# vankxr/qo-100-tools

Hardware: AMD Instinct MI355X
Metric: complex-IQ MSamples/s through 255-tap FIR (higher is better)
Workload: dtype f32

## Files before the change

### include/if_fir_debug.h

```cpp
#ifndef IF_FIR_DEBUG_H
#define IF_FIR_DEBUG_H

#include "if_fir.h"

#ifdef __cplusplus
extern "C" {
#endif

uint8_t if_fir_time_device(if_fir_ctx_t *pCtx, const void *pDevIn, void *pDevOut, uint64_t ullSamples,
                           uint32_t ulWarmup, uint32_t ulReps, float *pfMsPerCall);
uint32_t if_fir_debug_stamps(if_fir_ctx_t *pCtx, uint64_t *pullOut, uint32_t ulWords);
#define IF_FIR_DEBUG_TABLE_FLOATS 21632u
uint32_t if_fir_debug_fft_tables(const float *pfTaps, uint32_t ulTaps, uint32_t bComplexTaps, uint32_t ulDecimation,
                                 uint32_t ulNcoDelta, float *pfOut, uint32_t ulOutFloats);
uint32_t if_fir_debug_fft_tables_bank(const float *pfTaps, uint32_t ulTaps, uint32_t bComplexTaps, uint32_t ulBank, uint32_t ulParity,
                                      float *pfOut, uint32_t ulOutFloats);
uint32_t if_fir_debug_bank_tail(uint32_t ulDecimation, uint32_t bOwnCentres);
uint8_t if_fir_debug_bank_plan(const uint32_t *pulSlots, uint32_t ulChannels, uint32_t *pulOut);
#define IF_FIR_DEBUG_ODD_TABLE_FLOATS 10496u
uint32_t if_fir_debug_fft_tables_odd(const float *pfTaps, uint32_t ulTaps, uint32_t bComplexTaps, uint32_t ulDecimation,
                                     uint32_t ulNcoDelta, float *pfOut, uint32_t ulOutFloats);
uint8_t if_fir_debug_fft_schedule(uint64_t ullBlocks, uint32_t ulWorkgroups, uint32_t bSingleOk, int64_t *pllOut);
uint8_t if_fir_debug_queue_faults(if_fir_ctx_t *pCtx, uint32_t *pulFaults);
uint32_t if_fir_mc_debug_plan(uint32_t ulWorld, uint32_t ulChannels, uint32_t ulRank, uint64_t ullSamples,
                              uint32_t ulInBytes, uint32_t ulTaps, uint32_t ulDecimation, uint64_t ullConsumed,
                              uint64_t ullChunk, uint64_t *pullOut, uint32_t ulMaxOps);

uint8_t if_fir_debug_interp_config(if_fir_interp_t *pCtx, uint32_t bForceFull, uint32_t ulGridLimit);
uint8_t if_fir_debug_interp_seek(if_fir_interp_t *pCtx, uint64_t ullSamples);
uint32_t if_fir_debug_interp_tables(const float *pfTaps, uint32_t ulTaps, uint32_t bComplexTaps, float *pfOut, uint32_t ulOutFloats);
uint8_t if_fir_debug_interp_plan(uint32_t ulTaps, uint32_t ulInterpolation, uint32_t *pulRows, uint32_t *pulHistLen,
                                 uint32_t *pbFftOk);
uint8_t if_fir_debug_combiner_config(if_fir_combiner_t *pCtx, uint32_t ulGridLimit);
uint8_t if_fir_debug_combiner_seek(if_fir_combiner_t *pCtx, uint64_t ullSamples);
uint32_t if_fir_debug_combiner_tables(const float *pfTaps, uint32_t ulTaps, uint32_t bComplexTaps, double dCentre, uint32_t *pulGrid,
                                      int32_t *plResidual, float *pfOut, uint32_t ulOutFloats);
uint8_t if_fir_debug_resamp_config(if_fir_resamp_t *pCtx, uint32_t ulGridLimit, uint32_t *pulTileOutputs);
uint8_t if_fir_debug_ddc_config(if_fir_ddc_t *pCtx, uint32_t ulGridLimit, uint32_t *pulTileOutputs, uint64_t ullPosition);
uint8_t if_fir_debug_duc_config(if_fir_duc_t *pCtx, uint32_t ulGridLimit, uint32_t *pulTileInputs, uint64_t ullPosition);
uint8_t if_fir_debug_psd_plan(const if_fir_psd_t *pCtx, uint64_t ullSamples, uint64_t *pullPlan);
uint8_t if_fir_debug_arb_config(if_fir_arb_t *pCtx, uint32_t ulGridLimit, uint32_t *pulTileOutputs, uint64_t ullPosition,
                                uint64_t ullTimeOffset);
uint8_t if_fir_debug_pfb_config(if_fir_pfb_t *pCtx, uint32_t ulGridLimit, uint32_t *pulGroupFrames, uint64_t ullPosition);

#ifdef __cplusplus
}
#endif
#endif
```

### qo-100-tools_amd/csrc/if_fir_fft_kernel.inc

```
template <int OVL_ROWS, bool DEC4, bool I16, bool NCO, int CHAN, bool DECN, bool ACC>
__global__ __launch_bounds__(512, 2) IF_FIR_LDS_SINGLE_READS void fir_fft_kernel(const f2v *__restrict__ in_, f2v *__restrict__ out,
                                                        const f2v *__restrict__ tables, const f2v *__restrict__ hist,
                                                        int HL, int64_t N, int32_t n0, int64_t M, int64_t nblocks,
                                                        int64_t nblocks_main, unsigned int *queue, unsigned long long *dbg, int32_t diag,
                                                        uint32_t nco_phi0, uint32_t nco_delta, chan_arg_t<CHAN> chan,
                                                        uint32_t qsel, void *__restrict__ hist_out,
                                                        int32_t decn, int32_t decn_n0, int64_t decn_m, int32_t in_shift)
{
    static_assert(!ACC || (tail_single(CHAN) && OVL_ROWS == 32), "accumulating store: single-channel pipelines, 32 overlap rows");
    static_assert(!DECN || (!DEC4 && CHAN == TAIL_FULL_OR_DEC4), "general decimation = the full-rate pipeline with a selecting store");
    static_assert(tail_valid(CHAN) && (CHAN == TAIL_FULL_OR_DEC4 || DEC4), "every named tail but the first is a decimating one");
    static_assert(tail_has_nco(CHAN) || !NCO, "channels at their own centres: no common offset on top; the decimate-by-4 bank takes no NCO either");
    static_assert(OVL_ROWS >= 4 || (!DEC4 && !ACC), "2 overlap rows: full-rate pipeline (D = 1, odd D) only");
    constexpr bool TAN = tail_wants_tan(CHAN, DEC4);
    constexpr bool TANF = !DEC4;
    constexpr int OVL = 64 * OVL_ROWS;
    constexpr int ISZ = I16 ? 4 : 8;
    const char *in = reinterpret_cast<const char *>(in_);
    constexpr int L = FFT_N - OVL;
    constexpr int LOUT = tail_lout(CHAN, DEC4, L);
    constexpr int EARLY_GROUPS = CHAN == TAIL_DEC4_SUB ? FFT_EARLY_GROUPS_SUB : FFT_EARLY_GROUPS;
    constexpr int LAUX = FFT_LOAD_AUX;
    constexpr int EDGE = OVL_ROWS;
    extern __shared__ __attribute__((aligned(16))) char smem[];
    const int lane = threadIdx.x & 63;
    const int wid = __builtin_amdgcn_readfirstlane(threadIdx.x >> 6);
    if ((diag & 512) && blockIdx.x == 0)
    {
        if (lane == 0)
            atomicAdd(queue + 4, 1u);
        return;
    }
    cf r[64];
    const bool both = (CHAN == TAIL_BANK8_ALL) && ((chan.sub & 2u) != 0u);
    auto rb = [&](int64_t b) -> int64_t { return (CHAN == TAIL_BANK8_ALL && both) ? (b >> 1) : b; };
    bool loaded = false;
    const bool ahead = wid < FFT_WAVES / 2;
    const bool single = (diag & 131072) != 0;
    int64_t blk = single ? (int64_t)wid * gridDim.x + blockIdx.x : (int64_t)blockIdx.x * FFT_WAVES + wid;
    {
// ... 187 lines not shown
        for (int i = 0; i < 4; i++)
        {
            cf t[16];
#pragma unroll
            for (int j = 0; j < 16; j++)
                t[j] = r[phys(i, j)];
            if constexpr (TAN || TANF)
            {
                fft16_tw<false, 4>(t, tw2 + i * 60 + (lane >> 4));
#pragma unroll
                for (int j = 0; j < 16; j++)
                    r[phys(i, j)] = t[j];
            }
            else
            {
            cf w2[15];
            lds_fetch<15, 16>(w2, tw2 + 16 + (lane & 15));
            fft16<false>(t);
#pragma unroll
            for (int j = 0; j < 16; j++)
            {
                if (j == 0)
                    r[phys(i, j)] = t[j];
                else
                {
                    r[phys(i, j)] = cmul_v<false>(t[j], w2[j - 1]);
                }
            }
            }
        }
        FFT_STAMP(3);
        exchange2(r, xa);
        FFT_STAMP(4);
        const int64_t blk_next = queue_take(dq, simd, nblocks_main, nblocks);
        const int64_t s0n = rb(blk_next) * L - OVL + n0 - in_shift;
        const bool next_fast = (blk_next < nblocks) && (s0n >= 0) && !(diag & 1);
        const srd_t nsrd = make_srd(in + (next_fast ? s0n : 0) * ISZ, next_fast ? (N - s0n) * ISZ : 0);
        const int64_t obase = rb(blk) * LOUT;
        const srd_t osrd = make_srd(out + obase, (diag & 2) ? 0 : (M - obase) * 8);
        if constexpr (NCO && (CHAN == TAIL_BANK16_ALL || CHAN == TAIL_BANK8_ALL))
        {
            const float2 pb = phasor(nco_phi0 + nco_delta * (uint32_t)obase);
            if (lane == 0)
                *reinterpret_cast<cf *>(smem + LDS_QNCO + wid * 8) = (cf){pb.x, pb.y};
        }
        if constexpr (tail_is_bank(CHAN))
        {
#include "if_fir_fft_tails_bank.inc"
        }
        else
        {
#include "if_fir_fft_tails_single.inc"
        }
        FFT_STAMP(7);
        dbg_it++;
        loaded = next_fast;
        blk = blk_next;
    }
#ifndef IF_FIR_FFT_STAMPS
    if (dbg && lane == 0)
    {
        unsigned long long *d = dbg + 4 * ((size_t)blockIdx.x * FFT_WAVES + wid);
        d[0] = st_r0;
        d[1] = __builtin_amdgcn_s_memrealtime();
        d[2] = st_c0;
        d[3] = __builtin_amdgcn_s_memtime();
    }
// ... 4 lines not shown
```

### qo-100-tools_amd/csrc/if_fir_fft_launch.inc

```
template <int OVL_ROWS, bool DEC4, bool I16, bool NCO, int CHAN, bool DECN, bool ACC>
static constexpr auto fft_kernel_of()
{
#ifdef IF_FIR_FFT_DEC2_UNIT
    static_assert(tail_in_dec2_units(CHAN), "the decimate-by-2 units hold the decimate-by-2 tails only");
#else
    static_assert(!tail_in_dec2_units(CHAN), "the decimate-by-2 tails live in the decimate-by-2 units (launch_fft_dec2_rows)");
#endif
    return &fir_fft_kernel<OVL_ROWS, DEC4, I16, NCO, CHAN, DECN, ACC>;
}
template <int ROWS>
hipError_t launch_fft_dec2_rows(const LaunchArgs &a, int tail, bool nco, bool acc);
template <int OVL_ROWS, bool DEC4, bool I16, bool NCO, int CHAN, bool DECN, bool ACC>
static hipError_t launch_fft_t(const LaunchArgs &a)
{
    auto kern = fft_kernel_of<OVL_ROWS, DEC4, I16, NCO, CHAN, DECN, ACC>();
    constexpr int L = FFT_N - 64 * OVL_ROWS;
    constexpr int LOUT = tail_lout(CHAN, DEC4, L);
    static DeviceSetup setup;
    int ncus = 0;
    {
        const hipError_t e = device_setup(setup, a.device, reinterpret_cast<const void *>(kern), FFT_LDS_BYTES, &ncus);
        if (e != hipSuccess)
            return e;
    }
    constexpr int F = tail_factor(CHAN, DEC4);
    ChanArgs ca = a.chan ? *a.chan : ChanArgs{};
    ca.sub = tail_sub_word(CHAN, DEC4, a.D, ca.sub);
    const bool both = CHAN == TAIL_BANK8_ALL && (ca.sub & 2u);
    const int64_t m_rate = DECN ? a.N : CHAN == TAIL_BANK8_ALL ? a.M : (a.M - 1) * (int64_t)ca.sub + 1;
    const int32_t n0_rate = DECN ? 0 : a.n0;
    const int64_t nblocks = (a.M > 0 ? (m_rate + LOUT - 1) / LOUT : 0) * (both ? 2 : 1);
    if (nblocks <= 0)
        return hipSuccess;
    const int64_t wgs_max = (a.grid_limit > 0 && a.grid_limit < ncus) ? a.grid_limit : ncus;
    const FftLaunchPlan plan = fft_launch_plan(nblocks, wgs_max, !both && !(a.diag & 262144),
                                               (a.diag & 256) ? 0 : Q_TAIL_MAX_ROUNDS);
    uint32_t qsel = 0;
    {
        const hipError_t e = fft_queue_select(a, &qsel);
        if (e != hipSuccess)
            return e;
    }
    chan_arg_t<CHAN> cak;
    if constexpr (tail_is_bank(CHAN))
        cak = ca;
    else
        cak.sub = ca.sub;
    hipLaunchKernelGGL(kern, dim3((unsigned)plan.wgs), dim3(512), FFT_LDS_BYTES, a.stream,
                       reinterpret_cast<const f2v *>(a.in), reinterpret_cast<f2v *>(a.out),
                       reinterpret_cast<const f2v *>(a.fft_tables), reinterpret_cast<const f2v *>(a.hist_full), a.hist_len, a.N,
                       n0_rate, m_rate, nblocks, plan.nblocks_main, (unsigned int *)a.queue,
                       (unsigned long long *)a.dbg, (int32_t)a.diag | (plan.single ? 131072 : 0),
                       DECN ? 0u - a.nco_word * a.nco_abs0 : nco_phi0(a),
                       DECN ? 0u - a.nco_word : 0u - a.nco_word * (uint32_t)F,
                       cak, qsel, a.hist_out, (int32_t)a.D, (int32_t)a.n0, a.M,
                       (int32_t)a.in_shift);
    return fft_queue_launched(a);
}

enum { NCO_NEVER, NCO_BOTH, NCO_ALWAYS };
template <int ROWS, bool DEC4, int CHAN, bool DECN = false, bool ACC = false, int FORMS = tail_has_nco(CHAN) ? NCO_BOTH : NCO_NEVER>
static hipError_t launch_fft_form(const LaunchArgs &a, bool nco = false)
{
    static_assert(FORMS == NCO_NEVER || tail_has_nco(CHAN), "this tail has no NCO instantiation");
    if constexpr (FORMS == NCO_BOTH)
        switch ((a.in_i16 ? 2 : 0) | (nco ? 1 : 0))
        {
        case 0: return launch_fft_t<ROWS, DEC4, false, false, CHAN, DECN, ACC>(a);
        case 1: return launch_fft_t<ROWS, DEC4, false, true, CHAN, DECN, ACC>(a);
        case 2: return launch_fft_t<ROWS, DEC4, true, false, CHAN, DECN, ACC>(a);
        default: return launch_fft_t<ROWS, DEC4, true, true, CHAN, DECN, ACC>(a);
        }
    else
        return a.in_i16 ? launch_fft_t<ROWS, DEC4, true, FORMS == NCO_ALWAYS, CHAN, DECN, ACC>(a)
                        : launch_fft_t<ROWS, DEC4, false, FORMS == NCO_ALWAYS, CHAN, DECN, ACC>(a);
}

#ifdef IF_FIR_FFT_DEC2_UNIT
template <int ROWS>
hipError_t launch_fft_dec2_rows(const LaunchArgs &a, int tail, bool nco, bool acc)
{
    const bool plain = tail == TAIL_DEC2;
    if constexpr (ROWS == 32)
        if (acc)
            return plain ? launch_fft_form<ROWS, true, TAIL_DEC2, false, true>(a, nco) : launch_fft_form<ROWS, true, TAIL_DEC2_SUB, false, true>(a, nco);
    if (acc)
        return hipErrorInvalidConfiguration;
    return plain ? launch_fft_form<ROWS, true, TAIL_DEC2>(a, nco) : launch_fft_form<ROWS, true, TAIL_DEC2_SUB>(a, nco);
}
#if defined(IF_FIR_FFT_ONLY)
__attribute__((used)) static auto *const if_fir_fft_only_kernel = &fir_fft_kernel<IF_FIR_FFT_ONLY>;
#elif defined(IF_FIR_FFT_HAZARD_PROBE)
template __global__ void fir_fft_kernel<IF_FIR_FFT_ROWS, true, false, false, TAIL_DEC2, false, false>(
    const f2v *, f2v *, const f2v *, const f2v *, int, int64_t, int32_t, int64_t, int64_t, int64_t, unsigned int *,
    unsigned long long *, int32_t, uint32_t, uint32_t, chan_arg_t<TAIL_DEC2>, uint32_t, void *, int32_t, int32_t, int64_t, int32_t);
#else
template hipError_t launch_fft_dec2_rows<IF_FIR_FFT_ROWS>(const LaunchArgs &a, int tail, bool nco, bool acc);
#endif
#else
template <int ROWS>
static hipError_t launch_fft_bank8(const LaunchArgs &a, const FftRoute &r)
{
    bool general = a.chan->general || r.sub != 1;
    for (uint32_t c = 0; c < a.chan->count; c++)
        general = general || (a.chan->bin[c] & 255u) || a.chan->pword[c] != (a.chan->bin[c] << 20) + a.nco_word;
    if (general)
        return launch_fft_form<ROWS, true, TAIL_BANK8_CHANNEL, false, false, NCO_ALWAYS>(a);
    const bool nco = a.nco_word != 0;
    const ChanArgs &cin = *a.chan;
    uint32_t pmask[2], rest = 0;
    fft_bank8_plan(cin.slot, cin.count, a.fft_tables_b != nullptr && !(a.diag & 4096), pmask, &rest);
    bool first = true;
    const auto all_slots = [&](uint32_t mask, uint32_t sub, const void *tables) -> hipError_t {
        ChanArgs cs{};
        cs.count = (uint32_t)__builtin_popcount(mask);
        cs.sub = sub;
        cs.rot_e = cin.abs0n0 & 15u;
        cs.abs0n0 = cin.abs0n0;
        cs.mask16 = mask;
        for (uint32_t c = 0; c < cin.count; c++)
            if ((mask >> (cin.slot[c] & 15u)) & 1u)
                cs.out[cin.slot[c] & 15u] = cin.out[c];
        LaunchArgs p = a;
        p.chan = &cs;
        p.fft_tables = tables;
        if (!first)
            p.hist_out = nullptr;
        first = false;
// ... 109 lines not shown
```

### qo-100-tools_amd/csrc/if_fir_fft_queue.h

```cpp
#pragma once
#include <stdint.h>

#if defined(__HIPCC__)
#define IF_FIR_Q_FN __host__ __device__ inline __attribute__((always_inline))
#else
#define IF_FIR_Q_FN inline __attribute__((always_inline))
#endif

namespace if_fir
{

constexpr unsigned QB = 8;
constexpr unsigned Q_AHEAD = 2;
constexpr unsigned Q_RING = 4;
constexpr unsigned Q_SPIN_LIMIT = 1u << 22;
constexpr int64_t Q_NONE = (int64_t)1 << 46;

IF_FIR_Q_FN unsigned long long queue_word(unsigned global_group, unsigned local_group, unsigned slot)
{
    return ((unsigned long long)global_group << 32) | ((unsigned long long)(local_group & 0xffffffu) << 8) | slot;
}
IF_FIR_Q_FN unsigned long long queue_entry(unsigned global_group, unsigned local_group)
{
    return ((unsigned long long)global_group << 32) | local_group;
// ... 30 lines not shown
    queue_fetch(p, Q_AHEAD);
}

template <class P>
IF_FIR_Q_FN int64_t queue_tail(P &p, unsigned simd, int64_t nblocks_main, int64_t nblocks)
{
    if (p.tail_claim(simd) != 0)
        return Q_NONE;
    unsigned long long w = p.tail_add();
    if ((w & 0xffu) == 0)
    {
        const unsigned t = p.tail_ticket();
        w = ((unsigned long long)(4u * t + 1u) << 32) | 1u;
        p.tail_store(w);
    }
    else
    {
        unsigned spin = 0;
        for (; spin < Q_SPIN_LIMIT && (w >> 32) == 0; spin++)
        {
            p.pause();
            w = p.tail_load();
        }
        if ((w >> 32) == 0)
        {
            p.fault();
            return Q_NONE;
        }
    }
    const int64_t blk = nblocks_main + (int64_t)((unsigned)(w >> 32) - 1u) + simd;
    return blk < nblocks ? blk : Q_NONE;
}

template <class P>
IF_FIR_Q_FN int64_t queue_take(P &p, unsigned simd, int64_t nblocks_main, int64_t nblocks, unsigned *local_group = nullptr)
{
    for (unsigned spin = 0; spin < Q_SPIN_LIMIT; spin++)
    {
        const unsigned long long w = p.cur_add();
        const unsigned gg = (unsigned)(w >> 32), g = (unsigned)(w >> 8) & 0xffffffu, j = (unsigned)w & 0xffu;
        if (j < QB)
        {
            if (j == 0)
                queue_fetch(p, g + Q_AHEAD);
            if (j == QB - 1)
            {
                unsigned long long e;
                if (queue_wait_entry(p, g + 1, e))
                    p.cur_store(queue_word((unsigned)(e >> 32), g + 1, 0));
            }
            if (local_group)
                *local_group = g;
            const int64_t blk = (int64_t)gg * QB + j;
            if (blk < nblocks_main)
                return blk;
            return nblocks_main < nblocks ? queue_tail(p, simd, nblocks_main, nblocks) : Q_NONE;
        }
        if ((int64_t)gg * QB + QB - 1 >= nblocks_main)
            return nblocks_main < nblocks ? queue_tail(p, simd, nblocks_main, nblocks) : Q_NONE;
        for (; spin < Q_SPIN_LIMIT; spin++)
        {
            const unsigned long long c = p.cur_load();
            if (((unsigned)(c >> 8) & 0xffffffu) != g)
                break;
            p.pause();
        }
    }
    p.fault();
    return Q_NONE;
}

constexpr int64_t Q_TAIL_MAX_ROUNDS = 6;
IF_FIR_Q_FN int64_t queue_main_blocks(int64_t nblocks, int64_t wgs, int64_t max_rounds = Q_TAIL_MAX_ROUNDS)
{
    const int64_t simds = 4 * wgs, p = nblocks / (2 * simds), rem = nblocks - 2 * p * simds;
    return (p >= 1 && p <= max_rounds && rem > 0 && rem <= simds) ? 2 * p * simds : nblocks;
}

struct FftLaunchPlan
{
    int64_t wgs;
    int64_t nblocks_main;
    int64_t tickets;
    bool single;
};
IF_FIR_Q_FN FftLaunchPlan fft_launch_plan(int64_t nblocks, int64_t wgs_max, bool single_ok, int64_t tail_rounds)
{
    const int64_t groups = (nblocks + QB - 1) / QB;
    FftLaunchPlan p;
    p.single = single_ok && nblocks <= (int64_t)QB * wgs_max;
    const int64_t want = p.single ? nblocks : groups;
    p.wgs = want < wgs_max ? want : wgs_max;
    if (p.wgs < 1)
        p.wgs = 1;
    p.nblocks_main = p.single ? nblocks : queue_main_blocks(nblocks, p.wgs, tail_rounds);
    p.tickets = groups + 2 * p.wgs;
    return p;
}

IF_FIR_Q_FN unsigned long long queue_cur_init(unsigned wg, unsigned wgs, bool static_first)
{
    return static_first ? queue_word(wgs + wg, 1, 0) : queue_word(wg, 0, 0);
}
IF_FIR_Q_FN unsigned long long queue_ring_init(unsigned i, unsigned wg, unsigned wgs)
{
    return i < Q_AHEAD ? queue_entry(i * wgs + wg, i) : ~0ull;
}

}
```

### qo-100-tools_amd/csrc/if_fir_shim.cpp

```cpp
#include <hip/hip_runtime.h>

#include <cmath>
#include <cstdarg>
#include <cstdio>
#include <cstdlib>
#include <cstring>
#include <new>

#include "if_fir.h"
#ifdef IF_FIR_DEVELOPMENT
#include "if_fir_debug.h"
#endif
#include "if_fir_kernels.h"
#ifdef IF_FIR_DEVELOPMENT
#include "if_fir_fft_queue.h"
#endif

#define IF_FIR_API extern "C" __attribute__((visibility("default")))

struct Tuning
{
    int schedule;
    uint32_t diag;
    int grid_limit;
    bool no_fold;
    bool inject_failure;
    bool needs_debug;
};
static Tuning decode_tuning(uint32_t v)
{
    Tuning t{};
    t.schedule = v <= 6 ? (int)v : 0;
    t.diag = (v >= 1000 && v < 2000) ? v - 1000 : (v >= 1000000 && v < 3000000) ? v - 1000000 : 0;
    t.grid_limit = (v > 2000 && v < 3000) ? (int)(v - 2000) : 0;
    t.no_fold = v == 3000;
    t.inject_failure = v == 4000;
    t.needs_debug = (v >= 1000 && v < 2000) || v == 4000 || v >= 1000000;
    return t;
}

struct if_fir_ctx
{
    int device;
    hipStream_t own_stream;
    hipStream_t stream;
    int T, D;
    int ctaps;
    int in_i16;
    uint32_t backend_req;
    uint32_t backend;
    Tuning tuning;
    float *d_taps;
    void *d_hist[2];
    int hist_len;
    int hist_cur;
    uint64_t consumed;
    uint64_t max_samples;
    void *d_stage_in;
    void *d_stage_out;
    hipStream_t copy_in, copy_out;
    hipEvent_t *chunk_ev;
    uint32_t chunk_ev_count;
    float tone[10];
    float *h_taps;
    uint32_t nco_word;
    float *h_eff;
    void *d_fft_tables;
// ... 30 lines not shown
    } while (0)

static inline int eff_ctaps(const if_fir_ctx *ctx) { return ctx->ctaps || ctx->nco_word; }
static inline const float *eff_taps(const if_fir_ctx *ctx) { return ctx->h_eff ? ctx->h_eff : ctx->h_taps; }

static inline if_fir::FftRoute ctx_route(const if_fir_ctx *ctx, bool no_fold) { return if_fir::fft_route(ctx->T, ctx->D, if_fir::FFT_NO_BANK, ctx->nco_word != 0, no_fold); }

static uint32_t resolve_backend(const if_fir_ctx *ctx, uint32_t req)
{
    if (req != IF_FIR_BACKEND_AUTO)
        return req;
    if (if_fir::fft_supported(ctx->T, ctx->D))
        return IF_FIR_BACKEND_HIP_FFT;
    if (eff_ctaps(ctx) || ctx->in_i16)
        return IF_FIR_BACKEND_HIP_GENERIC;
    return if_fir::direct_supported(ctx->T, ctx->D) ? IF_FIR_BACKEND_HIP_DIRECT : IF_FIR_BACKEND_HIP_TAPSPLIT;
}

static int hist_len_for(int T, int D)
{
    const int need = T > 1 ? T - 1 : 0;
    const int a = if_fir::fft_route(T, D, if_fir::FFT_NO_BANK, false, false).hist_need, b = if_fir::fft_route(T, D, if_fir::FFT_NO_BANK, false, true).hist_need;
    return need > a && need > b ? need : a > b ? a : b;
}

#ifdef IF_FIR_DEVELOPMENT
static bool debug_enabled()
{
    const char *e = getenv("IF_FIR_DEBUG");
    return e && *e && *e != '0';
}
static uint32_t retired_diag_bits(uint32_t v)
{
    return decode_tuning(v).diag & ~(1u | 2u | 256u | 512u | 4096u | 8192u | 131072u | 262144u);
}
#endif

static bool backend_ok(const if_fir_ctx *ctx, uint32_t b)
{
    if ((eff_ctaps(ctx) || ctx->in_i16) && b != IF_FIR_BACKEND_HIP_FFT && b != IF_FIR_BACKEND_HIP_GENERIC)
        return false;
    switch (b)
    {
    case IF_FIR_BACKEND_HIP_DIRECT:
        return if_fir::direct_supported(ctx->T, ctx->D);
    case IF_FIR_BACKEND_HIP_GENERIC:
    case IF_FIR_BACKEND_HIP_TAPSPLIT:
        return true;
    case IF_FIR_BACKEND_HIP_FFT:
        return if_fir::fft_supported(ctx->T, ctx->D);
    default:
        return false;
    }
}

static uint8_t ensure_tables(if_fir_ctx *ctx, void **dst, const if_fir::FftRoute &route, const char *what)
{
    if (*dst)
        return 1;
    if_fir::FftImage image = route.image;
    float *tab = (float *)malloc(sizeof(float) * (size_t)image.floats);
    if (!tab)
    {
        set_err(ctx, "%s tables: out of host memory", what);
        return 0;
    }
    const double scale = ctx->in_i16 ? 0x1p-15 : 1.0;
// ... 761 lines not shown
                                                uint32_t ulNcoDelta, float *pfOut, uint32_t ulOutFloats)
{
    int F = 1;
    if (!pfTaps || !pfOut || !if_fir::fft_odd_tail((int)ulTaps, (int)ulDecimation, &F, nullptr, nullptr) ||
        ulOutFloats < (uint32_t)if_fir::fft_odd_table_floats(F))
        return 0;
    if_fir::fft_build_tables_odd(pfTaps, (int)ulTaps, bComplexTaps ? 1 : 0, F, ulNcoDelta, 1.0, pfOut);
    return (uint32_t)if_fir::fft_odd_table_floats(F);
}

IF_FIR_API uint8_t if_fir_debug_queue_faults(if_fir_ctx_t *pCtx, uint32_t *pulFaults)
{
    if (!pCtx || !pulFaults)
        return 0;
    HIP_TRY(pCtx, hipSetDevice(pCtx->device));
    HIP_TRY(pCtx, hipStreamSynchronize(pCtx->stream));
    HIP_TRY(pCtx, hipMemcpy(pulFaults, static_cast<const char *>(pCtx->d_queue) + 16, 4, hipMemcpyDeviceToHost));
    return 1;
}

IF_FIR_API uint8_t if_fir_debug_fft_schedule(uint64_t ullBlocks, uint32_t ulWorkgroups, uint32_t bSingleOk, int64_t *pllOut)
{
    if (!pllOut || !ullBlocks || !ulWorkgroups)
        return 0;
    const if_fir::FftLaunchPlan p =
        if_fir::fft_launch_plan((int64_t)ullBlocks, (int64_t)ulWorkgroups, bSingleOk != 0, if_fir::Q_TAIL_MAX_ROUNDS);
    pllOut[0] = p.wgs;
    pllOut[1] = p.nblocks_main;
    pllOut[2] = p.single ? 1 : 0;
    pllOut[3] = p.tickets;
    return 1;
}

#endif

IF_FIR_API uint8_t if_fir_power_device(if_fir_ctx_t *pCtx, const void *pDevIQ, uint64_t ullSamples, double *pdMeanPower)
{
    if (!pCtx || !pdMeanPower)
        return 0;
    *pdMeanPower = 0.0;
    if (ullSamples == 0)
        return 1;
    if (!pDevIQ || ((uintptr_t)pDevIQ & 15))
    {
        set_err(pCtx, "if_fir_power_device: the buffer must be a 16-byte aligned device pointer");
        return 0;
    }
    HIP_TRY(pCtx, hipSetDevice(pCtx->device));
    if (!pCtx->d_power)
        HIP_TRY(pCtx, hipMalloc(&pCtx->d_power, sizeof(double)));
    HIP_TRY(pCtx, if_fir::launch_power(pDevIQ, ullSamples, (double *)pCtx->d_power, pCtx->stream));
    double sum = 0.0;
    HIP_TRY(pCtx, hipMemcpyAsync(&sum, pCtx->d_power, sizeof(double), hipMemcpyDeviceToHost, pCtx->stream));
    HIP_TRY(pCtx, hipStreamSynchronize(pCtx->stream));
    *pdMeanPower = sum / (double)ullSamples;
    return 1;
}

IF_FIR_API uint8_t if_fir_host_alloc(if_fir_ctx_t *pCtx, void **ppHost, uint64_t ullBytes)
{
    if (!pCtx || !ppHost)
        return 0;
    *ppHost = nullptr;
    HIP_TRY(pCtx, hipSetDevice(pCtx->device));
    HIP_TRY(pCtx, hipHostMalloc(ppHost, ullBytes ? ullBytes : 16, hipHostMallocDefault));
    return 1;
// ... 281 lines not shown
```

### qo-100-tools_amd/if_fir.py

```python
import ctypes
import os

import numpy as np

_HERE = os.path.dirname(os.path.abspath(__file__))
LIB_PATH = os.path.join(_HERE, "libif_fir.so")
DEV_LIB_PATH = os.path.join(_HERE, "libif_fir_dev.so")

INPUT_F32, INPUT_I16 = 0, 1
OUTPUT_F32, OUTPUT_I16 = 0, 1
BACKEND_AUTO, BACKEND_HIP_DIRECT, BACKEND_HIP_TAPSPLIT, BACKEND_HIP_GENERIC, BACKEND_HIP_FFT = range(5)
WINDOW_RECT, WINDOW_HAMMING, WINDOW_HANN, WINDOW_BLACKMAN = range(4)

EXPORTS = [
    "if_bpf_design", "if_bpf_design_complex", "if_fir_init", "if_fir_init_complex", "if_fir_destroy", "if_fir_reset", "if_fir_set_backend", "if_fir_get_backend",
    "if_fir_set_tuning", "if_fir_set_input_format", "if_fir_set_stream", "if_fir_synchronize", "if_fir_last_error", "if_fir_out_count",
    "if_fir_process", "if_fir_process_device", "if_fir_synth_device", "if_fir_dev_alloc",
    "if_fir_dev_free", "if_fir_dev_upload", "if_fir_dev_download", "if_fir_device_info",
    "if_fir_set_nco", "if_fir_get_nco", "if_fir_channelizer_process_device", "if_fir_channelizer_process_device_freq", "if_fir_host_alloc", "if_fir_host_free",
    "if_fir_power_device",
    "if_fir_mc_owner", "if_fir_mc_unique_id", "if_fir_mc_init", "if_fir_mc_destroy", "if_fir_mc_reset",
    "if_fir_mc_set_input_format", "if_fir_mc_process_device", "if_fir_mc_channel_ctx", "if_fir_mc_last_error",
    "if_fir_mc_set_chunk_samples", "if_fir_mc_get_chunk_samples",
    "if_fir_interp_init", "if_fir_interp_init_complex", "if_fir_interp_destroy", "if_fir_interp_reset", "if_fir_interp_set_backend",
    "if_fir_interp_get_backend", "if_fir_interp_set_input_format", "if_fir_interp_set_nco", "if_fir_interp_get_nco",
    "if_fir_interp_set_stream", "if_fir_interp_synchronize", "if_fir_interp_last_error", "if_fir_interp_out_count",
    "if_fir_interp_process", "if_fir_interp_process_device",
    "if_fir_resamp_init", "if_fir_resamp_init_complex", "if_fir_resamp_destroy", "if_fir_resamp_reset", "if_fir_resamp_set_input_format",
    "if_fir_resamp_set_stream", "if_fir_resamp_synchronize", "if_fir_resamp_last_error", "if_fir_resamp_out_count",
    "if_fir_resamp_process", "if_fir_resamp_process_device",
    "if_fir_psd_init", "if_fir_psd_destroy", "if_fir_psd_reset", "if_fir_psd_set_input_format", "if_fir_psd_set_stream",
    "if_fir_psd_synchronize", "if_fir_psd_last_error", "if_fir_psd_frame_count", "if_fir_psd_process", "if_fir_psd_process_device",
    "if_fir_combiner_init", "if_fir_combiner_init_complex", "if_fir_combiner_destroy", "if_fir_combiner_reset", "if_fir_combiner_set_backend",
    "if_fir_combiner_get_backend", "if_fir_combiner_set_input_format", "if_fir_combiner_set_centres", "if_fir_combiner_get_centres",
    "if_fir_combiner_set_stream", "if_fir_combiner_synchronize", "if_fir_combiner_last_error", "if_fir_combiner_out_count",
    "if_fir_combiner_process", "if_fir_combiner_process_device",
    "if_fir_ddc_init", "if_fir_ddc_init_complex", "if_fir_ddc_destroy", "if_fir_ddc_reset", "if_fir_ddc_set_input_format",
    "if_fir_ddc_set_nco", "if_fir_ddc_get_nco", "if_fir_ddc_set_stream", "if_fir_ddc_synchronize", "if_fir_ddc_last_error",
    "if_fir_ddc_out_count", "if_fir_ddc_process", "if_fir_ddc_process_device",
    "if_fir_duc_init", "if_fir_duc_init_complex", "if_fir_duc_destroy", "if_fir_duc_reset", "if_fir_duc_set_input_format",
    "if_fir_duc_set_output_format", "if_fir_duc_set_nco", "if_fir_duc_get_nco", "if_fir_duc_set_stream", "if_fir_duc_synchronize",
    "if_fir_duc_last_error", "if_fir_duc_out_count", "if_fir_duc_process", "if_fir_duc_process_device",
    "if_fir_arb_init", "if_fir_arb_destroy", "if_fir_arb_reset", "if_fir_arb_set_step", "if_fir_arb_set_input_format",
    "if_fir_arb_set_stream", "if_fir_arb_synchronize", "if_fir_arb_last_error", "if_fir_arb_out_count", "if_fir_arb_process",
    "if_fir_arb_process_device", "if_fir_arb_step_from_rates",
    "if_fir_pfb_init", "if_fir_pfb_destroy", "if_fir_pfb_reset", "if_fir_pfb_set_input_format", "if_fir_pfb_set_stream",
    "if_fir_pfb_synchronize", "if_fir_pfb_last_error", "if_fir_pfb_frame_count", "if_fir_pfb_process", "if_fir_pfb_process_device",
]
DEV_EXPORTS = ["if_fir_time_device", "if_fir_debug_stamps", "if_fir_debug_fft_tables", "if_fir_debug_fft_tables_odd", "if_fir_debug_fft_tables_bank",
               "if_fir_debug_bank_plan", "if_fir_debug_bank_tail", "if_fir_debug_fft_schedule",
               "if_fir_mc_debug_plan", "if_fir_debug_queue_faults",
               "if_fir_debug_interp_config", "if_fir_debug_interp_seek", "if_fir_debug_interp_tables", "if_fir_debug_interp_plan",
               "if_fir_debug_resamp_config", "if_fir_debug_psd_plan",
               "if_fir_debug_combiner_config", "if_fir_debug_combiner_seek", "if_fir_debug_combiner_tables",
               "if_fir_debug_ddc_config", "if_fir_debug_duc_config", "if_fir_debug_arb_config",
               "if_fir_debug_pfb_config"]
MC_ID_BYTES = 128


class PsdConfig(ctypes.Structure):
    _fields_ = [("ulSize", ctypes.c_uint32), ("ulHop", ctypes.c_uint32), ("ulSegments", ctypes.c_uint32), ("lFirstBin", ctypes.c_int32),
                ("ulBins", ctypes.c_uint32), ("fRefPower", ctypes.c_float), ("ulInputFormat", ctypes.c_uint32)]


class PfbConfig(ctypes.Structure):
    _fields_ = [("ulChannels", ctypes.c_uint32), ("ulHop", ctypes.c_uint32), ("lFirstBin", ctypes.c_int32), ("ulBins", ctypes.c_uint32)]


class IfFirError(RuntimeError):
    pass


_libs = {}


def lib():
    return _load(LIB_PATH, False)


def dev_lib():
    return _load(DEV_LIB_PATH, True)


# ... 168 lines not shown
        L.if_fir_debug_pfb_config.restype = u8
        L.if_fir_debug_combiner_config.argtypes = [vp, u32]
        L.if_fir_debug_combiner_config.restype = u8
        L.if_fir_debug_combiner_seek.argtypes = [vp, u64]
        L.if_fir_debug_combiner_seek.restype = u8
        L.if_fir_debug_combiner_tables.argtypes = [f32p, u32, u32, ctypes.c_double, ctypes.POINTER(u32), ctypes.POINTER(i32), f32p, u32]
        L.if_fir_debug_combiner_tables.restype = u32
        L.if_fir_debug_psd_plan.argtypes = [vp, u64, ctypes.POINTER(u64)]
        L.if_fir_debug_psd_plan.restype = u8
        L.if_fir_debug_resamp_config.argtypes = [vp, u32, ctypes.POINTER(u32)]
        L.if_fir_debug_resamp_config.restype = u8
        L.if_fir_debug_ddc_config.argtypes = [vp, u32, ctypes.POINTER(u32), u64]
        L.if_fir_debug_ddc_config.restype = u8
        L.if_fir_debug_duc_config.argtypes = [vp, u32, ctypes.POINTER(u32), u64]
        L.if_fir_debug_duc_config.restype = u8
        L.if_fir_debug_arb_config.argtypes = [vp, u32, ctypes.POINTER(u32), u64, u64]
        L.if_fir_debug_arb_config.restype = u8
        L.if_fir_debug_interp_config.argtypes = [vp, u32, u32]
        L.if_fir_debug_interp_config.restype = u8
        L.if_fir_debug_interp_seek.argtypes = [vp, u64]
        L.if_fir_debug_interp_seek.restype = u8
        L.if_fir_debug_interp_tables.argtypes = [f32p, u32, u32, f32p, u32]
        L.if_fir_debug_interp_tables.restype = u32
        L.if_fir_debug_interp_plan.argtypes = [u32, u32, ctypes.POINTER(u32), ctypes.POINTER(u32), ctypes.POINTER(u32)]
        L.if_fir_debug_interp_plan.restype = u8
        L.if_fir_time_device.argtypes = [vp, vp, vp, u64, u32, u32, f32p]
        L.if_fir_time_device.restype = u8
        L.if_fir_debug_stamps.argtypes = [vp, ctypes.POINTER(u64), u32]
        L.if_fir_debug_stamps.restype = u32
        L.if_fir_debug_fft_tables.argtypes = [f32p, u32, u32, u32, u32, f32p, u32]
        L.if_fir_debug_fft_tables.restype = u32
        L.if_fir_debug_fft_schedule.argtypes = [u64, u32, u32, ctypes.POINTER(ctypes.c_int64)]
        L.if_fir_debug_fft_schedule.restype = u8
        L.if_fir_mc_debug_plan.argtypes = [u32, u32, u32, u64, u32, u32, u32, u64, u64, ctypes.POINTER(u64), u32]
        L.if_fir_mc_debug_plan.restype = u32
        L.if_fir_debug_queue_faults.argtypes = [vp, ctypes.POINTER(u32)]
        L.if_fir_debug_queue_faults.restype = u8
    _libs[path] = L
    return L


def _f32p(a):
    return a.ctypes.data_as(ctypes.POINTER(ctypes.c_float))


def _taps_arg(taps, complex_taps):
    taps = np.asarray(taps)
    if np.iscomplexobj(taps):
        taps = np.ascontiguousarray(taps.astype(np.complex64)).view(np.float32)
        complex_taps = True
    taps = np.ascontiguousarray(taps, dtype=np.float32)
    return taps, (taps.size // 2 if complex_taps else taps.size), bool(complex_taps)


def bpf_design(taps, f_low=0.15, f_high=0.25, window=WINDOW_BLACKMAN):
    h = np.zeros(max(int(taps), 0), dtype=np.float32)
    if not lib().if_bpf_design(_f32p(h), int(taps), float(f_low), float(f_high), int(window)):
        raise IfFirError("if_bpf_design rejected taps=%r band=[%r,%r] window=%r" % (taps, f_low, f_high, window))
    return h


def bpf_design_complex(taps, centre=0.2, bandwidth=0.1, window=WINDOW_BLACKMAN):
    g = np.zeros(2 * max(int(taps), 0), dtype=np.float32)
    if not lib().if_bpf_design_complex(_f32p(g), int(taps), float(centre), float(bandwidth), int(window)):
        raise IfFirError("if_bpf_design_complex rejected taps=%r centre=%r bandwidth=%r" % (taps, centre, bandwidth))
    return g
# ... 745 lines not shown
    k = len(slots)
    arr = (ctypes.c_uint32 * k)(*[int(v) for v in slots])
    out = (ctypes.c_uint32 * 3)()
    L = dev_lib()
    L.if_fir_debug_bank_plan.restype = ctypes.c_uint8
    if not L.if_fir_debug_bank_plan(arr, ctypes.c_uint32(k), out):
        raise IfFirError("if_fir_debug_bank_plan: 1..16 channels")
    return int(out[0]), int(out[1]), [c for c in range(k) if (out[2] >> c) & 1]


def debug_fft_tables_odd(taps, decimation, complex_taps=False, nco_delta=0):
    taps = np.ascontiguousarray(taps, dtype=np.float32)
    t = taps.size // 2 if complex_taps else taps.size
    nfl = 10496 + 512
    out = np.zeros(nfl, dtype=np.float32)
    L = dev_lib()
    L.if_fir_debug_fft_tables_odd.restype = ctypes.c_uint32
    n = L.if_fir_debug_fft_tables_odd(_f32p(taps), ctypes.c_uint32(t), ctypes.c_uint32(1 if complex_taps else 0),
                                      ctypes.c_uint32(int(decimation)), ctypes.c_uint32(int(nco_delta) & 0xFFFFFFFF), _f32p(out),
                                      ctypes.c_uint32(out.size))
    if n != nfl:
        raise IfFirError("if_fir_debug_fft_tables_odd: (taps=%d, decimation=%d) is not served by the odd-decimation kernel" % (t, decimation))
    c = out.view(np.complex64)
    return {"g": c[0:3072], "tb": c[3072:3328], "tc": c[3328:4096], "twd": c[4096:5120], "twe": c[5120:5184], "ncob": c[5184:5248], "pht": c[5248:5504]}


def debug_fft_schedule(nblocks, workgroups=256, single_ok=True):
    out = (ctypes.c_int64 * 4)()
    if not dev_lib().if_fir_debug_fft_schedule(int(nblocks), int(workgroups), 1 if single_ok else 0, out):
        raise IfFirError("if_fir_debug_fft_schedule: bad arguments")
    return dict(zip(("wgs", "nblocks_main", "single", "tickets"), [int(v) for v in out]))


def mc_owner(channel, world):
    return int(lib().if_fir_mc_owner(int(channel), int(world)))


MC_CHUNK_UNIT = 215040
MC_NEVER_SPLIT = (1 << 64) - 1


def mc_debug_plan(world, channels, rank, samples, in_bytes=8, decimation=1, consumed=0, chunk=0, taps=255):
    n = dev_lib().if_fir_mc_debug_plan(int(world), int(channels), int(rank), int(samples), int(in_bytes), int(taps),
                                       int(decimation), int(consumed), int(chunk), None, 0)
    buf = np.zeros(8 * max(n, 1), dtype=np.uint64)
    dev_lib().if_fir_mc_debug_plan(int(world), int(channels), int(rank), int(samples), int(in_bytes), int(taps), int(decimation),
                                   int(consumed), int(chunk), buf.ctypes.data_as(ctypes.POINTER(ctypes.c_uint64)), n)
    keys = ("kind", "phase", "group", "peer", "channel", "chunk", "offset", "bytes")
    return [dict(zip(keys, (int(v) for v in buf[8 * i:8 * i + 8]))) for i in range(n)]


def mc_unique_id():
    buf = (ctypes.c_uint8 * MC_ID_BYTES)()
    if not lib().if_fir_mc_unique_id(buf):
        raise IfFirError(lib().if_fir_mc_last_error(None).decode())
    return bytes(buf)


class IfFirMc:

    def __init__(self, taps, decimation, max_samples, device=0, rank=0, world=1, unique_id=None, dev=False):
        self._L = dev_lib() if dev else lib()
        taps = np.ascontiguousarray(np.asarray(taps, dtype=np.float32))
        if taps.ndim != 2:
            raise IfFirError("taps must be a (channels, taps) array")
        self.channels, self.rank, self.world = int(taps.shape[0]), int(rank), int(world)
# ... 63 lines not shown
```

Before: 600,300.

## Taper work-queue group sizes toward the end of the FFT block schedule

```diff
diff --git a/include/if_fir_debug.h b/include/if_fir_debug.h
--- a/include/if_fir_debug.h
+++ b/include/if_fir_debug.h
@@ -21,6 +21,8 @@
 uint32_t if_fir_debug_fft_tables_odd(const float *pfTaps, uint32_t ulTaps, uint32_t bComplexTaps, uint32_t ulDecimation,
                                      uint32_t ulNcoDelta, float *pfOut, uint32_t ulOutFloats);
 uint8_t if_fir_debug_fft_schedule(uint64_t ullBlocks, uint32_t ulWorkgroups, uint32_t bSingleOk, int64_t *pllOut);
+uint64_t if_fir_debug_fft_taper(uint64_t ullBlocks, uint32_t ulWorkgroups, uint32_t bSingleOk, uint32_t bTaperOk, int64_t *pllOut,
+                                int64_t *pllGroups, uint64_t ullMaxGroups);
 uint8_t if_fir_debug_queue_faults(if_fir_ctx_t *pCtx, uint32_t *pulFaults);
 uint32_t if_fir_mc_debug_plan(uint32_t ulWorld, uint32_t ulChannels, uint32_t ulRank, uint64_t ullSamples,
                               uint32_t ulInBytes, uint32_t ulTaps, uint32_t ulDecimation, uint64_t ullConsumed,
diff --git a/qo-100-tools_amd/csrc/if_fir_fft_kernel.inc b/qo-100-tools_amd/csrc/if_fir_fft_kernel.inc
--- a/qo-100-tools_amd/csrc/if_fir_fft_kernel.inc
+++ b/qo-100-tools_amd/csrc/if_fir_fft_kernel.inc
@@ -5,7 +5,8 @@
                                                         int64_t nblocks_main, unsigned int *queue, unsigned long long *dbg, int32_t diag,
                                                         uint32_t nco_phi0, uint32_t nco_delta, chan_arg_t<CHAN> chan,
                                                         uint32_t qsel, void *__restrict__ hist_out,
-                                                        int32_t decn, int32_t decn_n0, int64_t decn_m, int32_t in_shift)
+                                                        int32_t decn, int32_t decn_n0, int64_t decn_m, int32_t in_shift,
+                                                        uint32_t taper_g8, uint32_t taper_c)
 {
     static_assert(!ACC || (tail_single(CHAN) && OVL_ROWS == 32), "accumulating store: single-channel pipelines, 32 overlap rows");
     static_assert(!DECN || (!DEC4 && CHAN == TAIL_FULL_OR_DEC4), "general decimation = the full-rate pipeline with a selecting store");
@@ -259,7 +260,7 @@
         FFT_STAMP(3);
         exchange2(r, xa);
         FFT_STAMP(4);
-        const int64_t blk_next = queue_take(dq, simd, nblocks_main, nblocks);
+        const int64_t blk_next = queue_take_tapered(dq, QueueTaper{taper_g8, taper_c}, simd, nblocks_main, nblocks);
         const int64_t s0n = rb(blk_next) * L - OVL + n0 - in_shift;
         const bool next_fast = (blk_next < nblocks) && (s0n >= 0) && !(diag & 1);
         const srd_t nsrd = make_srd(in + (next_fast ? s0n : 0) * ISZ, next_fast ? (N - s0n) * ISZ : 0);
diff --git a/qo-100-tools_amd/csrc/if_fir_fft_launch.inc b/qo-100-tools_amd/csrc/if_fir_fft_launch.inc
--- a/qo-100-tools_amd/csrc/if_fir_fft_launch.inc
+++ b/qo-100-tools_amd/csrc/if_fir_fft_launch.inc
@@ -35,6 +35,7 @@
     const int64_t wgs_max = (a.grid_limit > 0 && a.grid_limit < ncus) ? a.grid_limit : ncus;
     const FftLaunchPlan plan = fft_launch_plan(nblocks, wgs_max, !both && !(a.diag & 262144),
                                                (a.diag & 256) ? 0 : Q_TAIL_MAX_ROUNDS);
+    const QueueTaper take = fft_taper_plan(nblocks, plan, !both && !(a.diag & 1024)).take();
     uint32_t qsel = 0;
     {
         const hipError_t e = fft_queue_select(a, &qsel);
@@ -54,7 +55,7 @@
                        DECN ? 0u - a.nco_word * a.nco_abs0 : nco_phi0(a),
                        DECN ? 0u - a.nco_word : 0u - a.nco_word * (uint32_t)F,
                        cak, qsel, a.hist_out, (int32_t)a.D, (int32_t)a.n0, a.M,
-                       (int32_t)a.in_shift);
+                       (int32_t)a.in_shift, take.g8, take.c);
     return fft_queue_launched(a);
 }
 
@@ -93,7 +94,8 @@
 #elif defined(IF_FIR_FFT_HAZARD_PROBE)
 template __global__ void fir_fft_kernel<IF_FIR_FFT_ROWS, true, false, false, TAIL_DEC2, false, false>(
     const f2v *, f2v *, const f2v *, const f2v *, int, int64_t, int32_t, int64_t, int64_t, int64_t, unsigned int *,
-    unsigned long long *, int32_t, uint32_t, uint32_t, chan_arg_t<TAIL_DEC2>, uint32_t, void *, int32_t, int32_t, int64_t, int32_t);
+    unsigned long long *, int32_t, uint32_t, uint32_t, chan_arg_t<TAIL_DEC2>, uint32_t, void *, int32_t, int32_t, int64_t, int32_t,
+    uint32_t, uint32_t);
 #else
 template hipError_t launch_fft_dec2_rows<IF_FIR_FFT_ROWS>(const LaunchArgs &a, int tail, bool nco, bool acc);
 #endif
diff --git a/qo-100-tools_amd/csrc/if_fir_fft_queue.h b/qo-100-tools_amd/csrc/if_fir_fft_queue.h
--- a/qo-100-tools_amd/csrc/if_fir_fft_queue.h
+++ b/qo-100-tools_amd/csrc/if_fir_fft_queue.h
@@ -86,18 +86,42 @@
     return blk < nblocks ? blk : Q_NONE;
 }
 
-template <class P>
-IF_FIR_Q_FN int64_t queue_take(P &p, unsigned simd, int64_t nblocks_main, int64_t nblocks, unsigned *local_group = nullptr)
+constexpr unsigned Q_NO_TAPER = 0xffffffffu;
+struct QueueTaper
+{
+    unsigned g8;
+    unsigned c;
+};
+IF_FIR_Q_FN void queue_group(const QueueTaper &t, unsigned gg, int64_t end, int64_t *first, unsigned *size)
+{
+    if (gg < t.g8)
+    {
+        *first = (int64_t)gg * QB;
+        *size = QB;
+        return;
+    }
+    const unsigned u = gg - t.g8, q = u / t.c, k = q < QB - 1 ? q : QB - 1;
+    const int64_t f = (int64_t)t.g8 * QB + (int64_t)t.c * (QB * k - k * (k - 1) / 2) + (int64_t)(u - k * t.c) * (QB - k);
+    *first = f;
+    *size = f < end ? QB - k : QB;
+}
+
+template <class P>
+IF_FIR_Q_FN int64_t queue_take_tapered(P &p, const QueueTaper &taper, unsigned simd, int64_t nblocks_main, int64_t nblocks,
+                                       unsigned *local_group = nullptr)
 {
     for (unsigned spin = 0; spin < Q_SPIN_LIMIT; spin++)
     {
         const unsigned long long w = p.cur_add();
         const unsigned gg = (unsigned)(w >> 32), g = (unsigned)(w >> 8) & 0xffffffu, j = (unsigned)w & 0xffu;
-        if (j < QB)
+        int64_t first;
+        unsigned size;
+        queue_group(taper, gg, nblocks_main, &first, &size);
+        if (j < size)
         {
             if (j == 0)
                 queue_fetch(p, g + Q_AHEAD);
-            if (j == QB - 1)
+            if (j == size - 1)
             {
                 unsigned long long e;
                 if (queue_wait_entry(p, g + 1, e))
@@ -105,12 +129,12 @@
             }
             if (local_group)
                 *local_group = g;
-            const int64_t blk = (int64_t)gg * QB + j;
+            const int64_t blk = first + j;
             if (blk < nblocks_main)
                 return blk;
             return nblocks_main < nblocks ? queue_tail(p, simd, nblocks_main, nblocks) : Q_NONE;
         }
-        if ((int64_t)gg * QB + QB - 1 >= nblocks_main)
+        if (first + size - 1 >= nblocks_main)
             return nblocks_main < nblocks ? queue_tail(p, simd, nblocks_main, nblocks) : Q_NONE;
         for (; spin < Q_SPIN_LIMIT; spin++)
         {
@@ -122,6 +146,12 @@
     }
     p.fault();
     return Q_NONE;
+}
+
+template <class P>
+IF_FIR_Q_FN int64_t queue_take(P &p, unsigned simd, int64_t nblocks_main, int64_t nblocks, unsigned *local_group = nullptr)
+{
+    return queue_take_tapered(p, QueueTaper{Q_NO_TAPER, 1u}, simd, nblocks_main, nblocks, local_group);
 }
 
 constexpr int64_t Q_TAIL_MAX_ROUNDS = 6;
@@ -152,6 +182,33 @@
     return p;
 }
 
+struct FftTaperPlan
+{
+    bool on;
+    int64_t g8;
+    int64_t c;
+    int64_t groups;
+    int64_t tickets;
+    QueueTaper take() const { return on ? QueueTaper{(unsigned)g8, (unsigned)c} : QueueTaper{Q_NO_TAPER, 1u}; }
+};
+IF_FIR_Q_FN FftTaperPlan fft_taper_plan(int64_t nblocks, const FftLaunchPlan &lp, bool allowed)
+{
+    constexpr int64_t per_c = QB * (QB + 1) / 2;
+    FftTaperPlan t;
+    t.c = lp.wgs / (int64_t)QB > 1 ? lp.wgs / (int64_t)QB : 1;
+    t.g8 = nblocks >= per_c * t.c ? (nblocks - per_c * t.c) / (int64_t)QB : 0;
+    t.on = allowed && !lp.single && lp.nblocks_main == nblocks && t.g8 >= 3 * lp.wgs && t.g8 + 9 * t.c + 2 * lp.wgs < (int64_t)Q_NO_TAPER;
+    if (t.on)
+        t.groups = t.g8 + QB * t.c + (nblocks - QB * t.g8 - per_c * t.c);
+    else
+    {
+        t.groups = (nblocks + QB - 1) / QB;
+        t.g8 = t.groups;
+    }
+    t.tickets = t.groups + 2 * lp.wgs;
+    return t;
+}
+
 IF_FIR_Q_FN unsigned long long queue_cur_init(unsigned wg, unsigned wgs, bool static_first)
 {
     return static_first ? queue_word(wgs + wg, 1, 0) : queue_word(wg, 0, 0);
diff --git a/qo-100-tools_amd/csrc/if_fir_shim.cpp b/qo-100-tools_amd/csrc/if_fir_shim.cpp
--- a/qo-100-tools_amd/csrc/if_fir_shim.cpp
+++ b/qo-100-tools_amd/csrc/if_fir_shim.cpp
@@ -32,7 +32,9 @@
     Tuning t{};
     t.schedule = v <= 6 ? (int)v : 0;
     t.diag = (v >= 1000 && v < 2000) ? v - 1000 : (v >= 1000000 && v < 3000000) ? v - 1000000 : 0;
-    t.grid_limit = (v > 2000 && v < 3000) ? (int)(v - 2000) : 0;
+    t.grid_limit = (v > 2000 && v < 3000) ? (int)(v - 2000) : (v > 5000 && v < 6000) ? (int)(v - 5000) : 0;
+    if (v > 5000 && v < 6000)
+        t.diag = 1024u;
     t.no_fold = v == 3000;
     t.inject_failure = v == 4000;
     t.needs_debug = (v >= 1000 && v < 2000) || v == 4000 || v >= 1000000;
@@ -129,7 +131,7 @@
 }
 static uint32_t retired_diag_bits(uint32_t v)
 {
-    return decode_tuning(v).diag & ~(1u | 2u | 256u | 512u | 4096u | 8192u | 131072u | 262144u);
+    return decode_tuning(v).diag & ~(1u | 2u | 256u | 512u | 1024u | 4096u | 8192u | 131072u | 262144u);
 }
 #endif
 
@@ -957,6 +959,29 @@
     return 1;
 }
 
+IF_FIR_API uint64_t if_fir_debug_fft_taper(uint64_t ullBlocks, uint32_t ulWorkgroups, uint32_t bSingleOk, uint32_t bTaperOk, int64_t *pllOut,
+                                           int64_t *pllGroups, uint64_t ullMaxGroups)
+{
+    if (!pllOut || !ullBlocks || !ulWorkgroups)
+        return 0;
+    const if_fir::FftLaunchPlan p =
+        if_fir::fft_launch_plan((int64_t)ullBlocks, (int64_t)ulWorkgroups, bSingleOk != 0, if_fir::Q_TAIL_MAX_ROUNDS);
+    const if_fir::FftTaperPlan t = if_fir::fft_taper_plan((int64_t)ullBlocks, p, bTaperOk != 0);
+    pllOut[0] = t.on ? 1 : 0;
+    pllOut[1] = t.g8;
+    pllOut[2] = t.c;
+    pllOut[3] = t.groups;
+    pllOut[4] = t.tickets;
+    const if_fir::QueueTaper take = t.take();
+    for (uint64_t gg = 0; pllGroups && gg < (uint64_t)t.tickets && gg < ullMaxGroups; gg++)
+    {
+        unsigned size = 0;
+        if_fir::queue_group(take, (unsigned)gg, p.nblocks_main, &pllGroups[2 * gg], &size);
+        pllGroups[2 * gg + 1] = size;
+    }
+    return (uint64_t)t.tickets;
+}
+
 #endif
 
 IF_FIR_API uint8_t if_fir_power_device(if_fir_ctx_t *pCtx, const void *pDevIQ, uint64_t ullSamples, double *pdMeanPower)
diff --git a/qo-100-tools_amd/if_fir.py b/qo-100-tools_amd/if_fir.py
--- a/qo-100-tools_amd/if_fir.py
+++ b/qo-100-tools_amd/if_fir.py
@@ -48,7 +48,7 @@
     "if_fir_pfb_synchronize", "if_fir_pfb_last_error", "if_fir_pfb_frame_count", "if_fir_pfb_process", "if_fir_pfb_process_device",
 ]
 DEV_EXPORTS = ["if_fir_time_device", "if_fir_debug_stamps", "if_fir_debug_fft_tables", "if_fir_debug_fft_tables_odd", "if_fir_debug_fft_tables_bank",
-               "if_fir_debug_bank_plan", "if_fir_debug_bank_tail", "if_fir_debug_fft_schedule",
+               "if_fir_debug_bank_plan", "if_fir_debug_bank_tail", "if_fir_debug_fft_schedule", "if_fir_debug_fft_taper",
                "if_fir_mc_debug_plan", "if_fir_debug_queue_faults",
                "if_fir_debug_interp_config", "if_fir_debug_interp_seek", "if_fir_debug_interp_tables", "if_fir_debug_interp_plan",
                "if_fir_debug_resamp_config", "if_fir_debug_psd_plan",
@@ -283,6 +283,9 @@
         L.if_fir_debug_fft_tables.restype = u32
         L.if_fir_debug_fft_schedule.argtypes = [u64, u32, u32, ctypes.POINTER(ctypes.c_int64)]
         L.if_fir_debug_fft_schedule.restype = u8
+        if hasattr(L, "if_fir_debug_fft_taper"):
+            L.if_fir_debug_fft_taper.argtypes = [u64, u32, u32, u32, ctypes.POINTER(ctypes.c_int64), ctypes.POINTER(ctypes.c_int64), u64]
+            L.if_fir_debug_fft_taper.restype = u64
         L.if_fir_mc_debug_plan.argtypes = [u32, u32, u32, u64, u32, u32, u32, u64, u64, ctypes.POINTER(u64), u32]
         L.if_fir_mc_debug_plan.restype = u32
         L.if_fir_debug_queue_faults.argtypes = [vp, ctypes.POINTER(u32)]
@@ -1094,6 +1097,19 @@
     return dict(zip(("wgs", "nblocks_main", "single", "tickets"), [int(v) for v in out]))
 
 
+def debug_fft_taper(nblocks, workgroups=256, single_ok=True, taper_ok=True):
+    out = (ctypes.c_int64 * 5)()
+    args = (int(nblocks), int(workgroups), 1 if single_ok else 0, 1 if taper_ok else 0, out)
+    pairs = int(dev_lib().if_fir_debug_fft_taper(*args, None, 0))
+    if not pairs:
+        raise IfFirError("if_fir_debug_fft_taper: bad arguments")
+    groups = np.zeros(2 * pairs, dtype=np.int64)
+    dev_lib().if_fir_debug_fft_taper(*args, groups.ctypes.data_as(ctypes.POINTER(ctypes.c_int64)), pairs)
+    d = dict(zip(("on", "g8", "c", "groups", "tickets"), [int(v) for v in out]))
+    d["first"], d["size"] = groups[0::2].copy(), groups[1::2].copy()
+    return d
+
+
 def mc_owner(channel, world):
     return int(lib().if_fir_mc_owner(int(channel), int(world)))
 
```

After: 601,100 (median of 2 runs). About the same (+0.1%).
